# lgemc/WildlifeMapper

Measured on AMD Instinct MI355X. Metric: 1024x1024 tiles/sec (whole node), higher is better.
Workload: dtype fp16; 1 GPU; vit_h full path fft+encoder+decoder+PostProcess/NMS, fp16 MFMA, batch=16 tiles/GPU of 1024x1024x3 (BASELINE.json configs[2]); parallelism=dp1 tile shard, weights=seed 0 synthetic (random init), tolerance=logits within 1e-3 relative of the fp32 CPU forward, identical NMS index lists

## Files before the change

### include/wm_hip.h

```cpp
#ifndef WM_HIP_H
#define WM_HIP_H

#include <stdint.h>

#ifdef __cplusplus
extern "C" {
#endif

#define WM_ABI_VERSION 13

#define WM_PREC_BF16 0
#define WM_PREC_FP16 1
#define WM_PREC_FP8 2

#define WM_MAX_GLOBAL 8
#define WM_NUM_QUERIES 51
#define WM_NUM_LOGITS 8

typedef struct wm_config {
    int32_t embed_dim;
    int32_t depth;
    int32_t num_heads;
    int32_t num_global;
    int32_t global_attn_indexes[WM_MAX_GLOBAL];
// ... 236 lines not shown
                        float eps, void* out_16_dev, int M, int N, int K, int act, int precision, void* stream);
int wm_op_gemm16_stats(const void* a_dev, const void* w_dev, const float* bias_dev, const float* residual_dev, float* out_f32_dev,
                       void* x16_dev, float* stats_dev, int M, int N, int K, int layout, int precision, void* stream);
int wm_op_pack16(const void* in_dev, void* out_dev, int64_t rows, int K, void* stream);
int wm_op_unpack16(const void* in_dev, void* out_dev, int64_t rows, int K, void* stream);

int wm_op_ln_stats16_split(const float* x_dev, float* stats_dev, void* hi_dev, void* lo_dev, float* x_rw_dev, int64_t rows, int C,
                           int precision, void* stream);
int wm_op_gemm16_split(const void* a_dev, const void* w_dev, const float* bias_dev, void* hi_dev, void* lo_dev, float* stats_dev,
                       int M, int N, int K, int layout, int precision, void* stream);
int wm_op_stream_merge(const void* hi_dev, const void* lo_dev, float* out_dev, int64_t rows, int C, int precision, void* stream);

int wm_op_gemm8(const void* a_dev, const void* w_dev, const float* wscale_dev, const float* bias_dev,
                const float* residual_dev, float* out_f32_dev, void* out_16_dev, void* out_8_dev,
                int M, int N, int K, int act, int precision, void* stream);
int wm_op_stream_rows(float* x_f32_dev, void* hi_dev, void* lo_dev, int64_t rows, int C, int precision, int merge, void* stream);
int wm_op_gemm8_planes(const void* a_dev, const void* w_dev, const float* wscale_dev, const float* bias_dev, void* hi_dev, void* lo_dev,
                       int M, int N, int K, int precision, void* stream);
int wm_op_layernorm_fp8_plane(const void* hi_dev, const float* gamma_dev, const float* beta_dev, float eps, void* out_8_dev, int64_t rows, int C,
                              int precision, void* stream);
int wm_op_cvt_f32_to_fp8(const float* in_dev, void* out_dev, int64_t n, void* stream);

int wm_op_conv3x3_16(const void* a_dev, const void* w_dev, float* out_dev, int batch, int c_out, int c_in,
                     int precision, void* stream);

int wm_op_patch_embed16(const void* img16_dev, const void* w_dev, const float* bias_dev, float* out_f32_dev, void* out_16_dev,
                        int batch, int n_out, int c_in, int precision, void* stream);

#define WM_GEMM32_SPLIT 0x100
#define WM_GEMM32_PRESPLIT 0x200
int wm_op_gemm32(const float* a_dev, const float* w_dev, const float* bias_dev,
                 const float* residual_dev, float* out_dev, int M, int N, int K, int act, void* stream);

int wm_op_layernorm(const float* x_dev, const float* gamma_dev, const float* beta_dev, float eps,
                    float* out_f32_dev, void* out_16_dev, int64_t rows, int C, int precision, void* stream);

int wm_op_encoder_attention(const void* qkv_dev, const float* qkv_bias_dev,
                            const float* rel_pos_h_dev, const float* rel_pos_w_dev, void* out_dev,
                            int batch, int heads, int head_dim, int window, int precision, void* stream);

int wm_op_encoder_attention_qkv(const void* q_dev, const void* k_dev, const void* v_dev, int token_stride,
                                const float* qkv_bias_dev, const float* rel_pos_h_dev, const float* rel_pos_w_dev,
                                void* out_dev, int batch, int heads, int head_dim, int window, int precision, void* stream);

int wm_op_mha16(const void* q_dev, int q_stride, const void* k_dev, int k_stride,
                const void* v_dev, int v_stride, void* out_dev, int out_stride,
                int batch, int heads, int head_dim, int nq, int nk, int precision, void* stream);

int wm_op_mha32(const float* q_dev, const float* k_dev, const float* v_dev, float* out_dev,
                int batch, int heads, int head_dim, int nq, int nk, void* stream);

#ifdef __cplusplus
}
#endif
#endif
```

### wildlifemapper_amd/_native.py

```python
from __future__ import annotations

import ctypes as C
import os
from typing import Optional

import torch

_HERE = os.path.dirname(os.path.abspath(__file__))
LIB_PATH = os.environ.get("WM_HIP_LIB") or os.path.join(_HERE, "libwm_hip.so")

PREC_BF16, PREC_FP16, PREC_FP8 = 0, 1, 2
PREC_BY_NAME = {"bf16": PREC_BF16, "fp16": PREC_FP16, "f16": PREC_FP16, "fp8": PREC_FP8}
NUM_QUERIES, NUM_LOGITS = 51, 8
KCLASS_NAMES = ("gemm16", "attn_window", "attn_global", "layernorm", "other")
GEMM_VARIANTS = ("v1_128", "v2_160", "v2_128", "v3_lockstep", "v3_conv3x3", "v5_320", "v5_320_res", "v5_256", "v5_256_res",
                 "v5_320_lnf", "v5_256_lnf", "fp8_320", "fp8_256", "v5_320_foldp", "v5_256_foldp", "v5_320_split", "v5_256_split", "v3_patch_embed", "fp8_256_planes")
FLAG_CONF, FLAG_SCORE, FLAG_NMS, FLAG_MERGED = 1, 2, 4, 8
CRITERION_MAX_TARGETS, CRITERION_SUMS, CRITERION_NONFINITE, CRITERION_UNSOLVED = 2048, 8, 1, 2
CENSUS_MAX_DETS, CENSUS_SAME_CLASS, CENSUS_UNSOLVED = 262144, 1, 1
COVERAGE_MAX_SIDE, COVERAGE_MAX_CELLS, COVERAGE_MAX_FRAMES, COVERAGE_CLASSES, COVERAGE_STATS = 16384, 1 << 26, 65535, 7, 16
MOSAIC_NEAREST, MOSAIC_BILINEAR, MOSAIC_NORTH_UP = 0, 1, 1
MOSAIC_BAD_SLOT, MOSAIC_BAD_SIZE, MOSAIC_BAD_SOURCE = 1, 2, 4
REGISTER_MAX_SIDE, REGISTER_MAX_SEARCH, REGISTER_MAX_PAIRS = 512, 64, 65535
REGISTER_BAD_SLOT, REGISTER_BAD_SIZE, REGISTER_BAD_PAIR = 1, 2, 4
# ... 62 lines not shown
    "wm_criterion": (_I, [_P, _P, _P, _P, _P, C.POINTER(C.c_int32), _I, _F, _F, _F, _F, _P, _L, _P, _P, _P, _P, _P, _P, _P]),
    "wm_forward": (_I, [_P, _P, _P, _P, _P, _P, _I, _P]),
    "wm_set_tap": (_I, [_P, _I]),
    "wm_read_tap": (_I, [_P, _P, _I, _P]),
    "wm_profile_enable": (_I, [_P, _I]),
    "wm_profile_reset": (_I, [_P]),
    "wm_profile_read": (_I, [_P, C.POINTER(WmKclassStat)]),
    "wm_debug_gemm_variant_counts": (_I, [C.POINTER(_L), _I]),
    "wm_debug_reset_gemm_variant_counts": (_I, []),
    "wm_debug_saturation_enable": (_I, [_P, _I]),
    "wm_debug_saturation_read": (_I, [_P, C.POINTER(_L), _I, _I, _P]),
    "wm_op_cvt_f32_to_16": (_I, [_P, _P, _L, _I, _P]),
    "wm_op_cvt_16_to_f32": (_I, [_P, _P, _L, _I, _P]),
    "wm_op_gemm16": (_I, [_P, _P, _P, _P, _I, _P, _P, _I, _I, _I, _I, _I, _P]),
    "wm_op_gemm16_takes_packed": (_I, [_I, _I, _I]),
    "wm_op_pack16": (_I, [_P, _P, _L, _I, _P]),
    "wm_op_ln_stats16": (_I, [_P, _P, _P, _L, _I, _I, _P]),
    "wm_op_ln_stats16_split": (_I, [_P, _P, _P, _P, _P, _L, _I, _I, _P]),
    "wm_op_gemm16_split": (_I, [_P, _P, _P, _P, _P, _P, _I, _I, _I, _I, _I, _P]),
    "wm_op_stream_merge": (_I, [_P, _P, _P, _L, _I, _I, _P]),
    "wm_op_unpack16": (_I, [_P, _P, _L, _I, _P]),
    "wm_stream_overflow": (_I, [_P, _I]),
    "wm_op_fold_weight16": (_I, [_P, _P, _P, _P, _P, _P, _P, _I, _I, _I, _P]),
    "wm_op_gemm16_folded": (_I, [_P, _P, _P, _P, _P, _F, _P, _I, _I, _I, _I, _I, _P]),
    "wm_op_gemm16_stats": (_I, [_P, _P, _P, _P, _P, _P, _P, _I, _I, _I, _I, _I, _P]),
    "wm_op_gemm8": (_I, [_P, _P, _P, _P, _P, _P, _P, _P, _I, _I, _I, _I, _I, _P]),
    "wm_op_stream_rows": (_I, [_P, _P, _P, _L, _I, _I, _I, _P]),
    "wm_op_gemm8_planes": (_I, [_P, _P, _P, _P, _P, _P, _I, _I, _I, _I, _P]),
    "wm_op_layernorm_fp8_plane": (_I, [_P, _P, _P, _F, _P, _L, _I, _I, _P]),
    "wm_op_cvt_f32_to_fp8": (_I, [_P, _P, _L, _P]),
    "wm_op_conv3x3_16": (_I, [_P, _P, _P, _I, _I, _I, _I, _P]),
    "wm_op_patch_embed16": (_I, [_P, _P, _P, _P, _P, _I, _I, _I, _I, _P]),
    "wm_op_gemm32": (_I, [_P, _P, _P, _P, _P, _I, _I, _I, _I, _P]),
    "wm_op_layernorm": (_I, [_P, _P, _P, _F, _P, _P, _L, _I, _I, _P]),
    "wm_op_encoder_attention": (_I, [_P, _P, _P, _P, _P, _I, _I, _I, _I, _I, _P]),
    "wm_op_encoder_attention_qkv": (_I, [_P, _P, _P, _I, _P, _P, _P, _P, _I, _I, _I, _I, _I, _P]),
    "wm_op_mha16": (_I, [_P, _I, _P, _I, _P, _I, _P, _I, _I, _I, _I, _I, _I, _I, _P]),
    "wm_op_mha32": (_I, [_P, _P, _P, _P, _I, _I, _I, _I, _I, _P]),
}

_lib: Optional[C.CDLL] = None


def lib() -> C.CDLL:
    global _lib
    if _lib is None:
        if not os.path.exists(LIB_PATH):
            raise RuntimeError(
                f"{LIB_PATH} not found: build it with `python -c 'import __graft_entry__ as g; g.build()'` "
                "(hipcc --offload-arch=gfx950).  There is no CPU fallback.")
        l = C.CDLL(LIB_PATH)
        for name, (res, args) in SYMBOLS.items():
            fn = getattr(l, name)
            fn.restype = res
            fn.argtypes = args
        got = l.wm_abi_version()
        if got != ABI_VERSION:
            raise RuntimeError(f"{LIB_PATH} reports ABI version {got}, this binding was written for {ABI_VERSION}: "
                               "rebuild it (python -c 'import __graft_entry__ as g; g.build()')")
        _lib = l
    return _lib


def gemm_variant_counts(reset: bool = False) -> dict:
    arr = (C.c_int64 * len(GEMM_VARIANTS))()
    check(lib().wm_debug_gemm_variant_counts(arr, len(GEMM_VARIANTS)))
# ... 26 lines not shown
```

### wildlifemapper_amd/csrc/gemm32.h

```cpp
#pragma once
#include "wm_common.h"
#include "gemm_common.h"

namespace wm {

struct Gemm32Args {
    const float* A; const float* W; const float* bias; const float* residual; float* out;
    int M, N, K, act;
    int lda;
};

__global__ __launch_bounds__(256) void gemm32_kernel(Gemm32Args p) {
    constexpr int BM = 64, BN = 64, BK = 32, LD = BK + 1;
    __shared__ float sA[BM * LD];
    __shared__ float sW[BN * LD];
    const int tid = threadIdx.x, lane = tid & 63, wave = tid >> 6;
    const int wr = wave >> 1, wc = wave & 1;
    const int ntn = (p.N + BN - 1) / BN;
    const int lid = xcd_remap(blockIdx.x, gridDim.x);
    const int m0 = (lid / ntn) * BM, n0 = (lid % ntn) * BN;
    const int lrow = tid >> 2, lcol = (tid & 3) * 8;

    f32x16 acc;
#pragma unroll
// ... 126 lines not shown
        if (kt + 2 < nk) fetch(s, (kt + 2) * BK);
#pragma unroll
        for (int ks = 0; ks < 2; ++ks) {
            const typename FP16::vec8 a_hi = *(const typename FP16::vec8*)(sAh + fa + 16 * ks), a_lo = *(const typename FP16::vec8*)(sAl + fa + 16 * ks);
            const typename FP16::vec8 w_hi = *(const typename FP16::vec8*)(sWh + fw + 16 * ks), w_lo = *(const typename FP16::vec8*)(sWl + fw + 16 * ks);
            accx = FP16::mfma32(a_lo, w_hi, accx);
            accx = FP16::mfma32(a_hi, w_lo, accx);
            acc = FP16::mfma32(a_hi, w_hi, acc);
        }
    };
    for (int kt = 0; kt < nk; kt += 2) {
        step(st[0], kt);
        if (kt + 1 < nk) step(st[1], kt + 1);
    }
    if (amax >= 65504.f && p.overflow) *(volatile int*)p.overflow = 1;

    const int n = n0 + wc * 32 + (lane & 31);
    if (n >= p.N) return;
    const float bv = p.bias ? p.bias[n] : 0.f;
#pragma unroll
    for (int r = 0; r < 16; ++r) {
        const int m = m0 + wr * 32 + (r & 3) + 8 * (r >> 2) + 4 * (lane >> 5);
        if (m < p.M) {
            float v = (acc[r] + accx[r] * (1.0f / G32X3_LOSCALE)) * (1.0f / G32X3_WSCALE) + bv;
            if (p.act == ACT_RELU) v = fmaxf(v, 0.f);
            else if (p.act == ACT_GELU) v = gelu_erf(v);
            else if (p.act == ACT_SIGMOID) v = 1.0f / (1.0f + expf(-v));
            if (p.residual) v += p.residual[(size_t)m * p.N + n];
            p.out[(size_t)m * p.N + n] = v;
        }
    }
}

}
```

### wildlifemapper_amd/csrc/host_decoder.h

```cpp
#pragma once
#include "dec_kernels.h"
#include "host_encoder.h"

namespace {

struct DecAttnW { const float *wq, *bq, *wk, *bk, *wv, *bv, *wo, *bo; int internal; };

DecAttnW dec_w(wm_handle* h, const std::string& p, int internal) {
    return DecAttnW{W32(h, p + "q_proj.weight"), W32(h, p + "q_proj.bias"), W32(h, p + "k_proj.weight"), W32(h, p + "k_proj.bias"),
                    W32(h, p + "v_proj.weight"), W32(h, p + "v_proj.bias"), W32(h, p + "out_proj.weight"), W32(h, p + "out_proj.bias"), internal};
}

int decoder_impl(wm_handle* h, const float* keys_nhwc, float* logits, float* boxes, int B, hipStream_t s) {
    const std::string t = "mask_decoder.transformer.";
    const int E = OUTC, Mk = B * T, Mq = B * NQ;
    const float* tok = W32(h, "mask_decoder.mask_tokens.weight");
    float* keys = h->dkeys;
    HIP_TRY(hipMemcpyAsync(keys, keys_nhwc, (size_t)Mk * E * 4, hipMemcpyDeviceToDevice, s));
    float* queries = h->dq;
    WM_TRY(launch_simple(h, s, 0.0, add_bcast_kernel, dim3(grid_for((int64_t)Mq * E / 4)), dim3(256), (const float*)nullptr, tok, queries, (int64_t)Mq, E, NQ));

    auto add_q = [&](float* out) {
        return launch_simple(h, s, 0.0, add_bcast_kernel, dim3(grid_for((int64_t)Mq * E / 4)), dim3(256), (const float*)queries, tok, out, (int64_t)Mq, E, NQ);
    };
    auto add_k = [&](float* out) {
        return launch_simple(h, s, 0.0, add_bcast_kernel, dim3(grid_for((int64_t)Mk * E / 4)), dim3(256), (const float*)keys, (const float*)h->kpe, out, (int64_t)Mk, E, T);
    };
    auto ln = [&](float* x, const std::string& n, int rows) {
        return launch_layernorm(h, s, WM_PREC_FP16, x, W32(h, n + ".weight"), W32(h, n + ".bias"), 1e-5f, x, nullptr, rows, E);
    };
    auto token_to_image = [&](const DecAttnW& w, const float* kin) -> int {
        WM_TRY(add_q(h->dt_h1));
        WM_TRY(launch_gemm32(h, s, h->dt_h1, w.wq, w.bq, nullptr, h->dt_q, Mq, w.internal, E, ACT_NONE));
        WM_TRY(launch_gemm32(h, s, kin, w.wk, w.bk, nullptr, h->dk_a, Mk, w.internal, E, ACT_NONE));
        WM_TRY(launch_gemm32(h, s, keys, w.wv, w.bv, nullptr, h->dk_b, Mk, w.internal, E, ACT_NONE));
        WM_TRY(launch_mha32(h, s, h->dt_q, h->dk_a, h->dk_b, h->dt_att, B, 8, w.internal / 8, NQ, T));
        WM_TRY(launch_gemm32(h, s, h->dt_att, w.wo, w.bo, queries, queries, Mq, E, w.internal, ACT_NONE));
        return 0;
    };
    float* kpe_sum = h->n1;

    for (int i = 0; i < 2; ++i) {
        const std::string L = t + "layers." + std::to_string(i) + ".";
        {
            const DecAttnW w = dec_w(h, L + "self_attn.", E);
            const float* qin = queries;
            if (i != 0) { WM_TRY(add_q(h->dt_h1)); qin = h->dt_h1; }
            WM_TRY(launch_gemm32(h, s, qin, w.wq, w.bq, nullptr, h->dt_q, Mq, E, E, ACT_NONE));
            WM_TRY(launch_gemm32(h, s, qin, w.wk, w.bk, nullptr, h->dt_k, Mq, E, E, ACT_NONE));
            WM_TRY(launch_gemm32(h, s, queries, w.wv, w.bv, nullptr, h->dt_v, Mq, E, E, ACT_NONE));
            WM_TRY(launch_mha32(h, s, h->dt_q, h->dt_k, h->dt_v, h->dt_att, B, 8, E / 8, NQ, NQ));
            WM_TRY(launch_gemm32(h, s, h->dt_att, w.wo, w.bo, i == 0 ? nullptr : queries, queries, Mq, E, E, ACT_NONE));
            WM_TRY(ln(queries, L + "norm1", Mq));
        }
        WM_TRY(add_k(kpe_sum));
        WM_TRY(token_to_image(dec_w(h, L + "cross_attn_token_to_image.", E / 2), kpe_sum));
        WM_TRY(ln(queries, L + "norm2", Mq));
        WM_TRY(launch_gemm32(h, s, queries, W32(h, L + "mlp.lin1.weight"), W32(h, L + "mlp.lin1.bias"), nullptr, h->dt_hid, Mq, DEC_MLP, E, ACT_RELU));
        WM_TRY(launch_gemm32(h, s, h->dt_hid, W32(h, L + "mlp.lin2.weight"), W32(h, L + "mlp.lin2.bias"), queries, queries, Mq, E, DEC_MLP, ACT_NONE));
        WM_TRY(ln(queries, L + "norm3", Mq));
        {
            const DecAttnW w = dec_w(h, L + "cross_attn_image_to_token.", E / 2);
            WM_TRY(add_q(h->dt_h1));
            WM_TRY(launch_gemm32(h, s, kpe_sum, w.wq, w.bq, nullptr, h->dk_a, Mk, w.internal, E, ACT_NONE));
            WM_TRY(launch_gemm32(h, s, h->dt_h1, w.wk, w.bk, nullptr, h->dt_k, Mq, w.internal, E, ACT_NONE));
            WM_TRY(launch_gemm32(h, s, queries, w.wv, w.bv, nullptr, h->dt_v, Mq, w.internal, E, ACT_NONE));
            WM_TRY(launch_mha32(h, s, h->dk_a, h->dt_k, h->dt_v, h->dk_c, B, 8, w.internal / 8, T, NQ));
            WM_TRY(launch_gemm32(h, s, h->dk_c, w.wo, w.bo, keys, keys, Mk, E, w.internal, ACT_NONE));
            WM_TRY(ln(keys, L + "norm4", Mk));
        }
    }
    WM_TRY(add_k(kpe_sum));
    WM_TRY(token_to_image(dec_w(h, t + "final_attn_token_to_image.", E / 2), kpe_sum));
    WM_TRY(ln(queries, t + "norm_final_attn", Mq));

    const std::string c = "mask_decoder.class_embed.layers.", bb = "mask_decoder.bbox_embed.layers.";
    WM_TRY(launch_gemm32(h, s, queries, W32(h, c + "0.weight"), W32(h, c + "0.bias"), nullptr, h->dt_h1, Mq, E, E, ACT_RELU));
    WM_TRY(launch_gemm32(h, s, h->dt_h1, W32(h, c + "1.weight"), W32(h, c + "1.bias"), nullptr, h->dt_h2, Mq, E, E, ACT_RELU));
    WM_TRY(launch_gemm32(h, s, h->dt_h2, W32(h, c + "2.weight"), W32(h, c + "2.bias"), nullptr, logits, Mq, WM_NUM_LOGITS, E, ACT_NONE));
    WM_TRY(launch_gemm32(h, s, queries, W32(h, bb + "0.weight"), W32(h, bb + "0.bias"), nullptr, h->dt_h1, Mq, E, E, ACT_RELU));
    WM_TRY(launch_gemm32(h, s, h->dt_h1, W32(h, bb + "1.weight"), W32(h, bb + "1.bias"), nullptr, h->dt_h2, Mq, E, E, ACT_RELU));
    WM_TRY(launch_gemm32(h, s, h->dt_h2, W32(h, bb + "2.weight"), W32(h, bb + "2.bias"), nullptr, boxes, Mq, 4, E, ACT_SIGMOID));
    return 0;
}

int forward_impl(wm_handle* h, const float* x_dev, const float* target_sizes_dev, float* logits_dev, float* boxes_dev,
                 wm_box_record* records_dev, int batch, hipStream_t s) {
    WM_TRY(fft_impl(h, x_dev, h->hfc, batch, s, true));
    WM_TRY(encoder_impl(h, x_dev, h->hfc, nullptr, batch, s, true));
    WM_TRY(decoder_impl(h, h->emb_nhwc, h->logits, h->boxes, batch, s));
    const float* ts = target_sizes_dev ? target_sizes_dev : h->tsz_default;
    WM_TRY(launch_simple(h, s, 0.0, postprocess_nms_kernel, dim3(batch), dim3(64), (const float*)h->logits, (const float*)h->boxes, ts,
                         0.05f, 0.5f, 0.4f, h->records));
    if (logits_dev) HIP_TRY(hipMemcpyAsync(logits_dev, h->logits, (size_t)batch * NQ * WM_NUM_LOGITS * 4, hipMemcpyDeviceToDevice, s));
    if (boxes_dev) HIP_TRY(hipMemcpyAsync(boxes_dev, h->boxes, (size_t)batch * NQ * 16, hipMemcpyDeviceToDevice, s));
    if (records_dev) HIP_TRY(hipMemcpyAsync(records_dev, h->records, (size_t)batch * NQ * sizeof(wm_box_record), hipMemcpyDeviceToDevice, s));
    return 0;
}

}
```

### wildlifemapper_amd/csrc/host_gemm.h

```cpp
#pragma once
#include "gemm16.h"
#include "gemm16_v2.h"
#include "gemm16_v3.h"
#include "gemm16_v5.h"
#include "gemm32.h"
#include "gemm8.h"
#include "misc_kernels.h"
#include "host_core.h"

namespace {

double gemm16_flops(const Gemm16Args& a) { return 2.0 * a.M * (double)a.N * a.K; }
double gemm16_bytes(const Gemm16Args& a) {
    return 2.0 * ((double)a.M * a.K + (double)a.N * a.K) + (a.out32 ? 4.0 : 0.0) * a.M * a.N + (a.out16 ? 2.0 : 0.0) * a.M * a.N +
           (a.residual ? 4.0 * (double)(a.res_mod > 0 ? a.res_mod : a.M) * a.N : 0.0);
}

template <class Kern, class Args>
int launch_gemm_kernel(wm_handle* h, hipStream_t s, Kern kern, int grid, int threads, int lds, const Args& a, int variant, double flops, double bytes) {
    WM_TRY(set_max_lds((const void*)kern, lds));
    if (variant >= 0) count_variant(variant);
    Bracket br(h, s, WM_KCLASS_GEMM16, flops, bytes);
    hipLaunchKernelGGL(kern, dim3(grid), dim3(threads), lds, s, a);
    HIP_TRY(hipGetLastError());
    return 0;
}

template <class T16>
int launch_gemm16_t(wm_handle* h, hipStream_t s, const Gemm16Args& a) {
    return launch_gemm_kernel(h, s, gemm16_kernel<T16>, (a.M / G16_BM) * (a.N / G16_BN), 256, G16_LDS_BYTES, a, WM_GEMM_V1_128, gemm16_flops(a), gemm16_bytes(a));
}

template <class T16, int BN>
int launch_gemm16v2_t(wm_handle* h, hipStream_t s, const Gemm16Args& a) {
    return launch_gemm_kernel(h, s, gemm16v2_kernel<T16, BN>, (a.M / 256) * (a.N / BN), 512, G2<BN>::LDS, a, BN == 160 ? WM_GEMM_V2_160 : WM_GEMM_V2_128,
                              gemm16_flops(a), gemm16_bytes(a));
}

template <class T16, int BN, bool FOLDP, bool FOLDC, bool SPLIT, int NSLOT = 3>
int launch_gemm16v5_t(wm_handle* h, hipStream_t s, const Gemm16Args& a_in) {
    using G = G3<BN>;
// ... 133 lines not shown
    if (M % 4096 || N % 256 || Cin % 32) return fail("conv3x3: M=%d N=%d C=%d unsupported (M %% 4096, N %% 256, C %% 32)", M, N, Cin);
    const uint16_t* zero_page = nullptr;
    WM_TRY(zero_page_for_device(&zero_page));
    Gemm16Args a{};
    a.A = (const u16*)A; a.W = (const u16*)W; a.out32 = out32; a.M = M; a.N = N; a.K = 9 * Cin; a.act = ACT_NONE; a.conv_c = Cin; a.zero_page = (const u16*)zero_page;
    using G = G3<256>;
    count_variant(WM_GEMM_V3_CONV3X3);
    return by_type16(prec, [&](auto t) {
        return launch_gemm_kernel(h, s, gemm16v3_kernel<decltype(t), 256, ALoad::Conv3x3>, (M / 256) * (N / 256), G::THREADS, G::LDS, a, -1,
                                  2.0 * M * (double)N * 9 * Cin, 2.0 * ((double)M * Cin + 9.0 * N * Cin) + 4.0 * M * N);
    });
}

int launch_patch_embed16(wm_handle* h, hipStream_t s, int prec, const void* img16, const void* W, const float* bias, const float* res, int res_mod,
                         float* out32, void* out16, int B, int N, int Cin) {
    const int M = B * 4096, K = Cin * 256;
    if (B <= 0 || (N % 320 && N % 256) || Cin <= 0) return fail("patch_embed: B=%d N=%d Cin=%d unsupported (N %% 320 or N %% 256)", B, N, Cin);
    if (!out32 && !out16) return fail("patch_embed: no output");
    Gemm16Args a{};
    a.A = (const u16*)img16; a.W = (const u16*)W; a.bias = bias; a.residual = res; a.out32 = out32; a.out16 = (u16*)out16;
    a.M = M; a.N = N; a.K = K; a.res_mod = res_mod; a.act = ACT_NONE; a.conv_c = Cin;
    count_variant(WM_GEMM_V3_PATCH);
    const double bytes = 2.0 * ((double)M * K + (double)N * K) + (out32 ? 4.0 : 0.0) * M * N + (out16 ? 2.0 : 0.0) * M * N;
    return by_type16(prec, [&](auto t) {
        return by_tile_width(N, [&](auto bn) {
            constexpr int BN = decltype(bn)::value;
            using G = G3<BN>;
            return launch_gemm_kernel(h, s, gemm16v3_kernel<decltype(t), BN, ALoad::PatchEmbed>, (M / 256) * (N / BN), G::THREADS, G::LDS, a, -1,
                                      2.0 * M * (double)N * K, bytes);
        });
    });
}

int launch_gemm32(wm_handle* h, hipStream_t s, const float* A, const float* W, const float* bias, const float* res,
                  float* out, int M, int N, int K, int act, int lda = 0, int mode = 0) {
    if (K % 16) return fail("gemm32: K=%d must be a multiple of 16", K);
    static const bool f32_only = getenv("WM_GEMM32_F32") && atoi(getenv("WM_GEMM32_F32")) != 0;
    if ((mode == 2 || mode == 3) && K % 32) return fail("gemm32 (split form): K=%d must be a multiple of 32", K);
    if (mode == 2 || mode == 3 || (mode == 0 && h && !f32_only && K % 32 == 0)) {
        Gemm32x3Args a{A, W, nullptr, nullptr, bias, res, out, M, N, K, act, lda > 0 ? lda : K, h ? h->overflow + 1 : nullptr};
        if (mode == 3) {
            const size_t n = (size_t)N * K;
            void* pb = nullptr;
            WM_TRY(op_scratch(s, 3, n * 4, &pb));
            u16* hi = (u16*)pb;
            hipLaunchKernelGGL(split_w32_kernel, dim3(grid_for((int64_t)n / 4)), dim3(256), 0, s, W, hi, hi + n, (int64_t)n / 4, (int*)nullptr);
            HIP_TRY(hipGetLastError());
            a.Whi = hi; a.Wlo = hi + n;
        }
        if (mode == 0) {
            auto it = h->w32x3.find(W);
            if (it == h->w32x3.end()) {
                uint16_t *hi = nullptr, *lo = nullptr;
                const size_t n = (size_t)N * K;
                if (n % 4) return fail("gemm32: weight of %zu elements", n);
                WM_TRY(dalloc(h, &hi, n * 2)); WM_TRY(dalloc(h, &lo, n * 2));
                hipLaunchKernelGGL(split_w32_kernel, dim3(grid_for((int64_t)n / 4)), dim3(256), 0, s, W, (u16*)hi, (u16*)lo, (int64_t)n / 4, h->overflow + 1);
                HIP_TRY(hipGetLastError());
                it = h->w32x3.emplace(W, std::make_pair(hi, lo)).first;
            }
            a.Whi = (const u16*)it->second.first; a.Wlo = (const u16*)it->second.second;
        }
        Bracket br(h, s, WM_KCLASS_OTHER, 2.0 * M * (double)N * K, 4.0 * ((double)M * K + (double)M * N) + 4.0 * (double)N * K);
        const dim3 grid(((N + 63) / 64) * ((M + 63) / 64));
        if (mode == 0 || mode == 3) hipLaunchKernelGGL(gemm32x3_kernel<true>, grid, dim3(256), 0, s, a);
        else hipLaunchKernelGGL(gemm32x3_kernel<false>, grid, dim3(256), 0, s, a);
        HIP_TRY(hipGetLastError());
        return 0;
    }
    Gemm32Args a{A, W, bias, res, out, M, N, K, act, lda > 0 ? lda : K};
    Bracket br(h, s, WM_KCLASS_OTHER, 2.0 * M * (double)N * K, 4.0 * ((double)M * K + (double)N * K + (double)M * N));
    hipLaunchKernelGGL(gemm32_kernel, dim3(((N + 63) / 64) * ((M + 63) / 64)), dim3(256), 0, s, a);
    HIP_TRY(hipGetLastError());
    return 0;
}

}
```

### wildlifemapper_amd/csrc/wm_api.hip

```cpp
#include "host_core.h"
#if WM_DEV_TIMELINE
#include "host_dev_timeline.h"
#endif
#include "host_gemm.h"
#include "host_norm.h"
#include "host_attn.h"
#include "host_weights.h"
#include "host_encoder.h"
#include "host_decoder.h"
#include "host_frontend.h"
#include "host_criterion.h"

extern "C" const char* wm_last_error(void) { return g_err; }
extern "C" int wm_abi_version(void) { return WM_ABI_VERSION; }

extern "C" int wm_create(const wm_config* cfg, int device, wm_handle** out) {
    if (!cfg || !out) return fail("wm_create: null argument");
    if (cfg->embed_dim <= 0 || cfg->num_heads <= 0 || cfg->embed_dim % cfg->num_heads) return fail("wm_create: bad dims");
    if (cfg->depth <= 0 || cfg->depth > 64) return fail("wm_create: depth %d out of range", cfg->depth);
    if (cfg->max_batch <= 0) return fail("wm_create: max_batch must be positive");
    if (cfg->embed_dim % 256 || cfg->embed_dim > 1280) return fail("wm_create: embed_dim %d unsupported (multiple of 256, <= 1280)", cfg->embed_dim);
    const int hd = cfg->embed_dim / cfg->num_heads;
    if (hd != 64 && hd != 80) return fail("wm_create: head_dim %d unsupported (64 or 80)", hd);
    if (cfg->precision != WM_PREC_BF16 && cfg->precision != WM_PREC_FP16 && cfg->precision != WM_PREC_FP8) return fail("wm_create: bad precision");
// ... 430 lines not shown
                        hi_dev, lo_dev);
}

extern "C" int wm_op_layernorm_fp8_plane(const void* hi_dev, const float* gamma_dev, const float* beta_dev, float eps, void* out_8_dev, int64_t rows, int C,
                                        int precision, void* stream) {
    if (!hi_dev || !out_8_dev || !gamma_dev || !beta_dev) return fail("wm_op_layernorm_fp8_plane: null buffer");
    return launch_layernorm_plane8(nullptr, (hipStream_t)stream, precision, hi_dev, gamma_dev, beta_dev, eps, out_8_dev, rows, C);
}

extern "C" int wm_op_cvt_f32_to_fp8(const float* in_dev, void* out_dev, int64_t n, void* stream) {
    if (n % 4) return fail("cvt fp8: n must be a multiple of 4");
    return launch_simple(nullptr, (hipStream_t)stream, 0.0, cvt_f32_to_fp8_kernel, dim3(grid_for(n / 4)), dim3(256), in_dev, (unsigned char*)out_dev, n / 4);
}

extern "C" int wm_op_conv3x3_16(const void* a_dev, const void* w_dev, float* out_dev, int batch, int c_out, int c_in, int precision,
                               void* stream) {
    return launch_conv3x3_16(nullptr, (hipStream_t)stream, precision, a_dev, w_dev, out_dev, batch * 4096, c_out, c_in);
}

extern "C" int wm_op_patch_embed16(const void* img16_dev, const void* w_dev, const float* bias_dev, float* out_f32_dev, void* out_16_dev,
                                  int batch, int n_out, int c_in, int precision, void* stream) {
    if (!img16_dev || !w_dev) return fail("wm_op_patch_embed16: null buffer");
    return launch_patch_embed16(nullptr, (hipStream_t)stream, precision, img16_dev, w_dev, bias_dev, nullptr, 0, out_f32_dev, out_16_dev, batch, n_out, c_in);
}

extern "C" int wm_op_gemm32(const float* a_dev, const float* w_dev, const float* bias_dev, const float* residual_dev, float* out_dev,
                            int M, int N, int K, int act, void* stream) {
    const int split = (act & WM_GEMM32_SPLIT) != 0, presplit = (act & WM_GEMM32_PRESPLIT) != 0;
    if (split && presplit) return fail("wm_op_gemm32: WM_GEMM32_SPLIT and WM_GEMM32_PRESPLIT are exclusive");
    return launch_gemm32(nullptr, (hipStream_t)stream, a_dev, w_dev, bias_dev, residual_dev, out_dev, M, N, K, act & 0xff, 0,
                         presplit ? 3 : split ? 2 : 1);
}

extern "C" int wm_op_layernorm(const float* x_dev, const float* gamma_dev, const float* beta_dev, float eps, float* out_f32_dev,
                               void* out_16_dev, int64_t rows, int C, int precision, void* stream) {
    const int packed = (precision & WM_LAYOUT_PACKED) != 0;
    precision &= ~WM_LAYOUT_PACKED;
    if (!out_f32_dev && out_16_dev)
        return launch_layernorm_block(nullptr, (hipStream_t)stream, precision, x_dev, gamma_dev, beta_dev, eps, out_16_dev, rows, C, packed);
    if (packed) return fail("wm_op_layernorm: the LDS-image-order output exists for the 16-bit-only form");
    return launch_layernorm(nullptr, (hipStream_t)stream, precision, x_dev, gamma_dev, beta_dev, eps, out_f32_dev, out_16_dev, rows, C);
}

extern "C" int wm_op_encoder_attention(const void* qkv_dev, const float* qkv_bias_dev, const float* rel_pos_h_dev,
                                       const float* rel_pos_w_dev, void* out_dev, int batch, int heads, int head_dim, int window,
                                       int precision, void* stream) {
    return launch_encoder_attention(nullptr, (hipStream_t)stream, precision, qkv_dev, qkv_bias_dev, rel_pos_h_dev, rel_pos_w_dev, out_dev,
                                    batch, heads, head_dim, window);
}

extern "C" int wm_op_encoder_attention_qkv(const void* q_dev, const void* k_dev, const void* v_dev, int token_stride, const float* qkv_bias_dev,
                                           const float* rel_pos_h_dev, const float* rel_pos_w_dev, void* out_dev, int batch, int heads,
                                           int head_dim, int window, int precision, void* stream) {
    AttnExtra x;
    x.k_sep = k_dev; x.v_sep = v_dev; x.tok_stride = token_stride;
    return launch_encoder_attention(nullptr, (hipStream_t)stream, precision, q_dev, qkv_bias_dev, rel_pos_h_dev, rel_pos_w_dev, out_dev,
                                    batch, heads, head_dim, window, x);
}

extern "C" int wm_op_mha16(const void* q_dev, int q_stride, const void* k_dev, int k_stride, const void* v_dev, int v_stride,
                           void* out_dev, int out_stride, int batch, int heads, int head_dim, int nq, int nk, int precision, void* stream) {
    return launch_mha16(nullptr, (hipStream_t)stream, precision, q_dev, q_stride, k_dev, k_stride, v_dev, v_stride, out_dev, out_stride,
                        batch, heads, head_dim, nq, nk);
}

extern "C" int wm_op_mha32(const float* q_dev, const float* k_dev, const float* v_dev, float* out_dev, int batch, int heads,
// ... 4 lines not shown
```

Before: 173.2 tiles/s.

## Fuse positional-embedding add and norm4 LayerNorm into row-block fp32x3 decoder GEMMs

Adds a row-blocked split-fp16 GEMM kernel that covers the full N (128 or 256) per block. It can add a broadcast positional embedding to A while loading, and can apply LayerNorm to the output rows in the epilogue. The decoder now uses it for key projections, which drops the separate add_k kernels and the kpe_sum buffer. It also folds the norm4 LayerNorm into the output projection and removes the initial device-to-device copy of the keys. The decoder is a small part of the vit_h pipeline, so the gain is likely small, and the fused epilogue may change rounding slightly.

```diff
diff --git a/include/wm_hip.h b/include/wm_hip.h
--- a/include/wm_hip.h
+++ b/include/wm_hip.h
@@ -292,6 +292,11 @@
 int wm_op_gemm32(const float* a_dev, const float* w_dev, const float* bias_dev,
                  const float* residual_dev, float* out_dev, int M, int N, int K, int act, void* stream);
 
+int wm_op_gemm32_rows(const float* a_dev, const float* pos_dev, int pos_rows, const float* w_dev, const float* bias_dev,
+                      const float* residual_dev, float* out_dev, const float* ln_gamma_dev, const float* ln_beta_dev, float ln_eps,
+                      int M, int N, int K, int act, void* stream);
+int wm_op_gemm32_takes_rows(int M, int N, int K);
+
 int wm_op_layernorm(const float* x_dev, const float* gamma_dev, const float* beta_dev, float eps,
                     float* out_f32_dev, void* out_16_dev, int64_t rows, int C, int precision, void* stream);
 
diff --git a/wildlifemapper_amd/_native.py b/wildlifemapper_amd/_native.py
--- a/wildlifemapper_amd/_native.py
+++ b/wildlifemapper_amd/_native.py
@@ -118,6 +118,8 @@
     "wm_op_conv3x3_16": (_I, [_P, _P, _P, _I, _I, _I, _I, _P]),
     "wm_op_patch_embed16": (_I, [_P, _P, _P, _P, _P, _I, _I, _I, _I, _P]),
     "wm_op_gemm32": (_I, [_P, _P, _P, _P, _P, _I, _I, _I, _I, _P]),
+    "wm_op_gemm32_rows": (_I, [_P, _P, _I, _P, _P, _P, _P, _P, _P, _F, _I, _I, _I, _I, _P]),
+    "wm_op_gemm32_takes_rows": (_I, [_I, _I, _I]),
     "wm_op_layernorm": (_I, [_P, _P, _P, _F, _P, _P, _L, _I, _I, _P]),
     "wm_op_encoder_attention": (_I, [_P, _P, _P, _P, _P, _I, _I, _I, _I, _I, _P]),
     "wm_op_encoder_attention_qkv": (_I, [_P, _P, _P, _I, _P, _P, _P, _P, _I, _I, _I, _I, _I, _P]),
diff --git a/wildlifemapper_amd/csrc/gemm32.h b/wildlifemapper_amd/csrc/gemm32.h
--- a/wildlifemapper_amd/csrc/gemm32.h
+++ b/wildlifemapper_amd/csrc/gemm32.h
@@ -182,4 +182,170 @@
     }
 }
 
-}
+struct Gemm32RowsArgs {
+    const float* A; const float* pos; const u16* Whi; const u16* Wlo;
+    const float* bias; const float* residual; float* out;
+    const float* ln_g; const float* ln_b; float ln_eps;
+    int M, N, K, act, lda, pos_rows;
+    int* overflow;
+};
+
+template <int I, int N, class F>
+__device__ __forceinline__ void g32_static_for(F&& f) {
+    if constexpr (I < N) {
+        f(std::integral_constant<int, I>{});
+        g32_static_for<I + 1, N>(f);
+    }
+}
+
+template <int NJ>
+struct G32Rows {
+    static constexpr int BM = 64, BK = 32, LDH = BK + 8, N = 64 * NJ;
+    static constexpr int LDO = N + 4;
+    static constexpr int LOOP_BYTES = (2 * BM + 2 * N) * LDH * 2, EPI_BYTES = BM * LDO * 4;
+    static constexpr int LDS = LOOP_BYTES > EPI_BYTES ? LOOP_BYTES : EPI_BYTES;
+};
+
+template <int NJ, bool LN>
+__global__ __launch_bounds__(256, NJ == 2 ? 3 : 2) void gemm32x3_rows_kernel(Gemm32RowsArgs p) {
+    using G = G32Rows<NJ>;
+    constexpr int BM = G::BM, BK = G::BK, LDH = G::LDH, N = G::N, LDO = G::LDO;
+    static_assert(!LN || NJ == 4, "the fused LayerNorm is the 256-column form: one wave per row");
+    extern __shared__ __attribute__((aligned(16))) unsigned char g32r_lds[];
+    u16* const sAh = (u16*)g32r_lds;
+    u16* const sAl = sAh + BM * LDH;
+    u16* const sWh = sAl + BM * LDH;
+    u16* const sWl = sWh + N * LDH;
+    float* const sO = (float*)g32r_lds;
+    const int tid = threadIdx.x, lane = tid & 63, wave = tid >> 6;
+    const int wr = wave >> 1, wc = wave & 1;
+    const int m0 = blockIdx.x * BM;
+    const int lrow = tid >> 2, lcol = (tid & 3) * 8;
+
+    f32x16 acc[NJ], accx[NJ];
+#pragma unroll
+    for (int j = 0; j < NJ; ++j)
+#pragma unroll
+        for (int r = 0; r < 16; ++r) acc[j][r] = accx[j][r] = 0.f;
+    const float* ap = p.A + (size_t)(m0 + lrow) * p.lda + lcol;
+    const float* pp = p.pos ? p.pos + (size_t)((m0 + lrow) % p.pos_rows) * p.K + lcol : nullptr;
+    const size_t woff = (size_t)lrow * p.K + lcol;
+    struct AStage { f32x4 a0, a1, p0, p1; };
+    AStage st[2];
+    f16x8 wh[NJ], wl[NJ];
+    float amax = 0.f;
+    auto fetch_a = [&](AStage& s, int k0) {
+        s.a0 = *(const f32x4*)(ap + k0); s.a1 = *(const f32x4*)(ap + k0 + 4);
+        if (pp) { s.p0 = *(const f32x4*)(pp + k0); s.p1 = *(const f32x4*)(pp + k0 + 4); }
+    };
+    auto fetch_w = [&](int k0) {
+        g32_static_for<0, NJ>([&](auto ic) {
+            constexpr int i = decltype(ic)::value;
+            wh[i] = *(const f16x8*)(p.Whi + woff + (size_t)i * 64 * p.K + k0);
+            wl[i] = *(const f16x8*)(p.Wlo + woff + (size_t)i * 64 * p.K + k0);
+        });
+    };
+    auto split8 = [&](const f32x4& x0, const f32x4& x1, uint4& hi, uint4& lo) {
+        union { uint4 raw; typename FP16::vec4 h[2]; } uh, ul;
+#pragma unroll
+        for (int j = 0; j < 8; ++j) {
+            const float x = j < 4 ? x0[j] : x1[j - 4];
+            amax = fmaxf(amax, fabsf(x));
+            uh.h[j >> 2][j & 3] = FP16::from_f32_bounded(x);
+            ul.h[j >> 2][j & 3] = FP16::from_f32_bounded((x - FP16::to_f32(uh.h[j >> 2][j & 3])) * G32X3_LOSCALE);
+        }
+        hi = uh.raw; lo = ul.raw;
+    };
+    const int nk = p.K / BK;
+    fetch_a(st[0], 0);
+    fetch_w(0);
+    if (nk > 1) fetch_a(st[1], BK);
+    const int fa = (wr * 32 + (lane & 31)) * LDH + 8 * (lane >> 5), fw = (wc * NJ * 32 + (lane & 31)) * LDH + 8 * (lane >> 5);
+    auto step = [&](AStage& s, int kt) {
+        uint4 ah, al;
+        if (pp) split8(s.a0 + s.p0, s.a1 + s.p1, ah, al);
+        else split8(s.a0, s.a1, ah, al);
+        __syncthreads();
+        *(uint4*)(sAh + lrow * LDH + lcol) = ah; *(uint4*)(sAl + lrow * LDH + lcol) = al;
+        g32_static_for<0, NJ>([&](auto ic) {
+            constexpr int i = decltype(ic)::value;
+            *(f16x8*)(sWh + (i * 64 + lrow) * LDH + lcol) = wh[i];
+            *(f16x8*)(sWl + (i * 64 + lrow) * LDH + lcol) = wl[i];
+        });
+        __syncthreads();
+        if (kt + 1 < nk) fetch_w((kt + 1) * BK);
+        if (kt + 2 < nk) fetch_a(s, (kt + 2) * BK);
+#pragma unroll
+        for (int ks = 0; ks < 2; ++ks) {
+            const typename FP16::vec8 a_hi = *(const typename FP16::vec8*)(sAh + fa + 16 * ks), a_lo = *(const typename FP16::vec8*)(sAl + fa + 16 * ks);
+#pragma unroll
+            for (int j = 0; j < NJ; ++j) {
+                const typename FP16::vec8 w_hi = *(const typename FP16::vec8*)(sWh + fw + j * 32 * LDH + 16 * ks);
+                const typename FP16::vec8 w_lo = *(const typename FP16::vec8*)(sWl + fw + j * 32 * LDH + 16 * ks);
+                accx[j] = FP16::mfma32(a_lo, w_hi, accx[j]);
+                accx[j] = FP16::mfma32(a_hi, w_lo, accx[j]);
+                acc[j] = FP16::mfma32(a_hi, w_hi, acc[j]);
+            }
+        }
+    };
+    for (int kt = 0; kt < nk; kt += 2) {
+        step(st[0], kt);
+        if (kt + 1 < nk) step(st[1], kt + 1);
+    }
+    if (amax >= 65504.f && p.overflow) *(volatile int*)p.overflow = 1;
+
+    __syncthreads();
+#pragma unroll
+    for (int j = 0; j < NJ; ++j) {
+        const int n = (wc * NJ + j) * 32 + (lane & 31);
+        const float bv = p.bias ? p.bias[n] : 0.f;
+#pragma unroll
+        for (int r = 0; r < 16; ++r) {
+            const int row = wr * 32 + (r & 3) + 8 * (r >> 2) + 4 * (lane >> 5);
+            float v = (acc[j][r] + accx[j][r] * (1.0f / G32X3_LOSCALE)) * (1.0f / G32X3_WSCALE) + bv;
+            if (p.act == ACT_RELU) v = fmaxf(v, 0.f);
+            else if (p.act == ACT_GELU) v = gelu_erf(v);
+            else if (p.act == ACT_SIGMOID) v = 1.0f / (1.0f + expf(-v));
+            sO[row * LDO + n] = v;
+        }
+    }
+    constexpr int LPR = N / 4, RPI = 64 / LPR, NIT = 16 / RPI;
+    const int c0 = (lane % LPR) * 4, row0 = wave * 16 + lane / LPR;
+    f32x4 rv[NIT], g, b;
+    if (p.residual) {
+#pragma unroll
+        for (int it = 0; it < NIT; ++it) rv[it] = *(const f32x4*)(p.residual + (size_t)(m0 + row0 + it * RPI) * N + c0);
+    }
+    if constexpr (LN) {
+        g = *(const f32x4*)(p.ln_g + c0);
+        b = *(const f32x4*)(p.ln_b + c0);
+    }
+    __syncthreads();
+#pragma unroll
+    for (int it = 0; it < NIT; ++it) {
+        const int row = row0 + it * RPI;
+        const size_t o = (size_t)(m0 + row) * N + c0;
+        f32x4 v = *(const f32x4*)(sO + row * LDO + c0);
+        if (p.residual) v += rv[it];
+        if constexpr (LN) {
+            float sum = 0.f;
+            sum += (v[0] + v[1]) + (v[2] + v[3]);
+            const float mean = wave_sum(sum) * (1.0f / N);
+            float sq = 0.f;
+#pragma unroll
+            for (int j = 0; j < 4; ++j) {
+                const float d = v[j] - mean;
+                sq += d * d;
+            }
+            const float var = wave_sum(sq) * (1.0f / N);
+            const float rstd = 1.0f / sqrtf(var + p.ln_eps);
+            f32x4 y;
+#pragma unroll
+            for (int j = 0; j < 4; ++j) y[j] = (v[j] - mean) * rstd * g[j] + b[j];
+            v = y;
+        }
+        *(f32x4*)(p.out + o) = v;
+    }
+}
+
+}
diff --git a/wildlifemapper_amd/csrc/host_decoder.h b/wildlifemapper_amd/csrc/host_decoder.h
--- a/wildlifemapper_amd/csrc/host_decoder.h
+++ b/wildlifemapper_amd/csrc/host_decoder.h
@@ -15,31 +15,27 @@
     const std::string t = "mask_decoder.transformer.";
     const int E = OUTC, Mk = B * T, Mq = B * NQ;
     const float* tok = W32(h, "mask_decoder.mask_tokens.weight");
-    float* keys = h->dkeys;
-    HIP_TRY(hipMemcpyAsync(keys, keys_nhwc, (size_t)Mk * E * 4, hipMemcpyDeviceToDevice, s));
+    const float* keys = keys_nhwc;
     float* queries = h->dq;
     WM_TRY(launch_simple(h, s, 0.0, add_bcast_kernel, dim3(grid_for((int64_t)Mq * E / 4)), dim3(256), (const float*)nullptr, tok, queries, (int64_t)Mq, E, NQ));
 
     auto add_q = [&](float* out) {
         return launch_simple(h, s, 0.0, add_bcast_kernel, dim3(grid_for((int64_t)Mq * E / 4)), dim3(256), (const float*)queries, tok, out, (int64_t)Mq, E, NQ);
     };
-    auto add_k = [&](float* out) {
-        return launch_simple(h, s, 0.0, add_bcast_kernel, dim3(grid_for((int64_t)Mk * E / 4)), dim3(256), (const float*)keys, (const float*)h->kpe, out, (int64_t)Mk, E, T);
-    };
+    Gemm32RowsExtra with_pe;
+    with_pe.pos = h->kpe; with_pe.pos_rows = T; with_pe.pos_scratch = h->n1;
     auto ln = [&](float* x, const std::string& n, int rows) {
         return launch_layernorm(h, s, WM_PREC_FP16, x, W32(h, n + ".weight"), W32(h, n + ".bias"), 1e-5f, x, nullptr, rows, E);
     };
-    auto token_to_image = [&](const DecAttnW& w, const float* kin) -> int {
+    auto token_to_image = [&](const DecAttnW& w) -> int {
         WM_TRY(add_q(h->dt_h1));
         WM_TRY(launch_gemm32(h, s, h->dt_h1, w.wq, w.bq, nullptr, h->dt_q, Mq, w.internal, E, ACT_NONE));
-        WM_TRY(launch_gemm32(h, s, kin, w.wk, w.bk, nullptr, h->dk_a, Mk, w.internal, E, ACT_NONE));
-        WM_TRY(launch_gemm32(h, s, keys, w.wv, w.bv, nullptr, h->dk_b, Mk, w.internal, E, ACT_NONE));
+        WM_TRY(launch_gemm32_rows(h, s, keys, w.wk, w.bk, nullptr, h->dk_a, Mk, w.internal, E, ACT_NONE, with_pe));
+        WM_TRY(launch_gemm32_rows(h, s, keys, w.wv, w.bv, nullptr, h->dk_b, Mk, w.internal, E, ACT_NONE, Gemm32RowsExtra{}));
         WM_TRY(launch_mha32(h, s, h->dt_q, h->dk_a, h->dk_b, h->dt_att, B, 8, w.internal / 8, NQ, T));
         WM_TRY(launch_gemm32(h, s, h->dt_att, w.wo, w.bo, queries, queries, Mq, E, w.internal, ACT_NONE));
         return 0;
     };
-    float* kpe_sum = h->n1;
-
     for (int i = 0; i < 2; ++i) {
         const std::string L = t + "layers." + std::to_string(i) + ".";
         {
@@ -53,8 +49,7 @@
             WM_TRY(launch_gemm32(h, s, h->dt_att, w.wo, w.bo, i == 0 ? nullptr : queries, queries, Mq, E, E, ACT_NONE));
             WM_TRY(ln(queries, L + "norm1", Mq));
         }
-        WM_TRY(add_k(kpe_sum));
-        WM_TRY(token_to_image(dec_w(h, L + "cross_attn_token_to_image.", E / 2), kpe_sum));
+        WM_TRY(token_to_image(dec_w(h, L + "cross_attn_token_to_image.", E / 2)));
         WM_TRY(ln(queries, L + "norm2", Mq));
         WM_TRY(launch_gemm32(h, s, queries, W32(h, L + "mlp.lin1.weight"), W32(h, L + "mlp.lin1.bias"), nullptr, h->dt_hid, Mq, DEC_MLP, E, ACT_RELU));
         WM_TRY(launch_gemm32(h, s, h->dt_hid, W32(h, L + "mlp.lin2.weight"), W32(h, L + "mlp.lin2.bias"), queries, queries, Mq, E, DEC_MLP, ACT_NONE));
@@ -62,16 +57,17 @@
         {
             const DecAttnW w = dec_w(h, L + "cross_attn_image_to_token.", E / 2);
             WM_TRY(add_q(h->dt_h1));
-            WM_TRY(launch_gemm32(h, s, kpe_sum, w.wq, w.bq, nullptr, h->dk_a, Mk, w.internal, E, ACT_NONE));
+            WM_TRY(launch_gemm32_rows(h, s, keys, w.wq, w.bq, nullptr, h->dk_a, Mk, w.internal, E, ACT_NONE, with_pe));
             WM_TRY(launch_gemm32(h, s, h->dt_h1, w.wk, w.bk, nullptr, h->dt_k, Mq, w.internal, E, ACT_NONE));
             WM_TRY(launch_gemm32(h, s, queries, w.wv, w.bv, nullptr, h->dt_v, Mq, w.internal, E, ACT_NONE));
             WM_TRY(launch_mha32(h, s, h->dk_a, h->dt_k, h->dt_v, h->dk_c, B, 8, w.internal / 8, T, NQ));
-            WM_TRY(launch_gemm32(h, s, h->dk_c, w.wo, w.bo, keys, keys, Mk, E, w.internal, ACT_NONE));
-            WM_TRY(ln(keys, L + "norm4", Mk));
+            Gemm32RowsExtra norm4;
+            norm4.ln_g = W32(h, L + "norm4.weight"); norm4.ln_b = W32(h, L + "norm4.bias"); norm4.ln_eps = 1e-5f;
+            WM_TRY(launch_gemm32_rows(h, s, h->dk_c, w.wo, w.bo, keys, h->dkeys, Mk, E, w.internal, ACT_NONE, norm4));
+            keys = h->dkeys;
         }
     }
-    WM_TRY(add_k(kpe_sum));
-    WM_TRY(token_to_image(dec_w(h, t + "final_attn_token_to_image.", E / 2), kpe_sum));
+    WM_TRY(token_to_image(dec_w(h, t + "final_attn_token_to_image.", E / 2)));
     WM_TRY(ln(queries, t + "norm_final_attn", Mq));
 
     const std::string c = "mask_decoder.class_embed.layers.", bb = "mask_decoder.bbox_embed.layers.";
diff --git a/wildlifemapper_amd/csrc/host_gemm.h b/wildlifemapper_amd/csrc/host_gemm.h
--- a/wildlifemapper_amd/csrc/host_gemm.h
+++ b/wildlifemapper_amd/csrc/host_gemm.h
@@ -6,7 +6,9 @@
 #include "gemm32.h"
 #include "gemm8.h"
 #include "misc_kernels.h"
+#include "dec_kernels.h"
 #include "host_core.h"
+#include "host_norm.h"
 
 namespace {
 
@@ -206,6 +208,30 @@
     });
 }
 
+static int gemm32_w_planes(wm_handle* h, hipStream_t s, const float* W, int N, int K, const u16** whi, const u16** wlo) {
+    const size_t n = (size_t)N * K;
+    if (n % 4) return fail("gemm32: weight of %zu elements", n);
+    if (!h) {
+        void* pb = nullptr;
+        WM_TRY(op_scratch(s, 3, n * 4, &pb));
+        u16* hi = (u16*)pb;
+        hipLaunchKernelGGL(split_w32_kernel, dim3(grid_for((int64_t)n / 4)), dim3(256), 0, s, W, hi, hi + n, (int64_t)n / 4, (int*)nullptr);
+        HIP_TRY(hipGetLastError());
+        *whi = hi; *wlo = hi + n;
+        return 0;
+    }
+    auto it = h->w32x3.find(W);
+    if (it == h->w32x3.end()) {
+        uint16_t *hi = nullptr, *lo = nullptr;
+        WM_TRY(dalloc(h, &hi, n * 2)); WM_TRY(dalloc(h, &lo, n * 2));
+        hipLaunchKernelGGL(split_w32_kernel, dim3(grid_for((int64_t)n / 4)), dim3(256), 0, s, W, (u16*)hi, (u16*)lo, (int64_t)n / 4, h->overflow + 1);
+        HIP_TRY(hipGetLastError());
+        it = h->w32x3.emplace(W, std::make_pair(hi, lo)).first;
+    }
+    *whi = (const u16*)it->second.first; *wlo = (const u16*)it->second.second;
+    return 0;
+}
+
 int launch_gemm32(wm_handle* h, hipStream_t s, const float* A, const float* W, const float* bias, const float* res,
                   float* out, int M, int N, int K, int act, int lda = 0, int mode = 0) {
     if (K % 16) return fail("gemm32: K=%d must be a multiple of 16", K);
@@ -213,28 +239,7 @@
     if ((mode == 2 || mode == 3) && K % 32) return fail("gemm32 (split form): K=%d must be a multiple of 32", K);
     if (mode == 2 || mode == 3 || (mode == 0 && h && !f32_only && K % 32 == 0)) {
         Gemm32x3Args a{A, W, nullptr, nullptr, bias, res, out, M, N, K, act, lda > 0 ? lda : K, h ? h->overflow + 1 : nullptr};
-        if (mode == 3) {
-            const size_t n = (size_t)N * K;
-            void* pb = nullptr;
-            WM_TRY(op_scratch(s, 3, n * 4, &pb));
-            u16* hi = (u16*)pb;
-            hipLaunchKernelGGL(split_w32_kernel, dim3(grid_for((int64_t)n / 4)), dim3(256), 0, s, W, hi, hi + n, (int64_t)n / 4, (int*)nullptr);
-            HIP_TRY(hipGetLastError());
-            a.Whi = hi; a.Wlo = hi + n;
-        }
-        if (mode == 0) {
-            auto it = h->w32x3.find(W);
-            if (it == h->w32x3.end()) {
-                uint16_t *hi = nullptr, *lo = nullptr;
-                const size_t n = (size_t)N * K;
-                if (n % 4) return fail("gemm32: weight of %zu elements", n);
-                WM_TRY(dalloc(h, &hi, n * 2)); WM_TRY(dalloc(h, &lo, n * 2));
-                hipLaunchKernelGGL(split_w32_kernel, dim3(grid_for((int64_t)n / 4)), dim3(256), 0, s, W, (u16*)hi, (u16*)lo, (int64_t)n / 4, h->overflow + 1);
-                HIP_TRY(hipGetLastError());
-                it = h->w32x3.emplace(W, std::make_pair(hi, lo)).first;
-            }
-            a.Whi = (const u16*)it->second.first; a.Wlo = (const u16*)it->second.second;
-        }
+        if (mode == 0 || mode == 3) WM_TRY(gemm32_w_planes(mode == 0 ? h : nullptr, s, W, N, K, &a.Whi, &a.Wlo));
         Bracket br(h, s, WM_KCLASS_OTHER, 2.0 * M * (double)N * K, 4.0 * ((double)M * K + (double)M * N) + 4.0 * (double)N * K);
         const dim3 grid(((N + 63) / 64) * ((M + 63) / 64));
         if (mode == 0 || mode == 3) hipLaunchKernelGGL(gemm32x3_kernel<true>, grid, dim3(256), 0, s, a);
@@ -249,4 +254,53 @@
     return 0;
 }
 
-}
+struct Gemm32RowsExtra {
+    const float* pos = nullptr;
+    int pos_rows = 0;
+    float* pos_scratch = nullptr;
+    const float* ln_g = nullptr;
+    const float* ln_b = nullptr;
+    float ln_eps = 0.f;
+};
+static bool gemm32_takes_rows(int M, int N, int K) { return M >= 4096 && M % 128 == 0 && (N == 128 || N == 256) && K > 0 && K % 32 == 0; }
+static bool aligned16(const void* p) { return ((uintptr_t)p & 15) == 0; }
+
+int launch_gemm32_rows(wm_handle* h, hipStream_t s, const float* A, const float* W, const float* bias, const float* res, float* out,
+                       int M, int N, int K, int act, const Gemm32RowsExtra& x) {
+    if (x.pos && x.pos_rows <= 0) return fail("gemm32 (rows): pos_rows=%d", x.pos_rows);
+    if ((x.ln_g != nullptr) != (x.ln_b != nullptr)) return fail("gemm32 (rows): LayerNorm takes both gamma and beta");
+    if (x.ln_g && N != 256) return fail("gemm32 (rows): the LayerNorm option is for N = 256, not %d", N);
+    static const bool f32_only = getenv("WM_GEMM32_F32") && atoi(getenv("WM_GEMM32_F32")) != 0;
+    const bool ptrs = aligned16(A) && aligned16(x.pos) && aligned16(res) && aligned16(out) && aligned16(x.ln_g) && aligned16(x.ln_b);
+    if (gemm32_takes_rows(M, N, K) && ptrs && !(h && f32_only)) {
+        Gemm32RowsArgs a{A, x.pos, nullptr, nullptr, bias, res, out, x.ln_g, x.ln_b, x.ln_eps, M, N, K, act, K, x.pos_rows, h ? h->overflow + 1 : nullptr};
+        WM_TRY(gemm32_w_planes(h, s, W, N, K, &a.Whi, &a.Wlo));
+        auto go = [&](auto kern, int lds) {
+            WM_TRY(set_max_lds((const void*)kern, lds));
+            Bracket br(h, s, WM_KCLASS_OTHER, 2.0 * M * (double)N * K,
+                       4.0 * ((double)M * K + (double)M * N * (res ? 2.0 : 1.0) + (double)N * K + (x.pos ? (double)x.pos_rows * K : 0.0)));
+            hipLaunchKernelGGL(kern, dim3(M / 64), dim3(256), lds, s, a);
+            HIP_TRY(hipGetLastError());
+            return 0;
+        };
+        if (N == 128) return go(gemm32x3_rows_kernel<2, false>, G32Rows<2>::LDS);
+        return x.ln_g ? go(gemm32x3_rows_kernel<4, true>, G32Rows<4>::LDS) : go(gemm32x3_rows_kernel<4, false>, G32Rows<4>::LDS);
+    }
+    const float* a_in = A;
+    if (x.pos) {
+        float* sum = x.pos_scratch;
+        if (!sum) {
+            void* pb = nullptr;
+            WM_TRY(op_scratch(s, 4, (size_t)M * K * 4, &pb));
+            sum = (float*)pb;
+        }
+        if (K % 4) return fail("gemm32 (rows): K=%d", K);
+        WM_TRY(launch_simple(h, s, 0.0, add_bcast_kernel, dim3(grid_for((int64_t)M * K / 4)), dim3(256), A, x.pos, sum, (int64_t)M, K, x.pos_rows));
+        a_in = sum;
+    }
+    WM_TRY(launch_gemm32(h, s, a_in, W, bias, res, out, M, N, K, act, 0, h ? 0 : 3));
+    if (x.ln_g) WM_TRY(launch_layernorm(h, s, WM_PREC_FP16, out, x.ln_g, x.ln_b, x.ln_eps, out, nullptr, M, N));
+    return 0;
+}
+
+}
diff --git a/wildlifemapper_amd/csrc/wm_api.hip b/wildlifemapper_amd/csrc/wm_api.hip
--- a/wildlifemapper_amd/csrc/wm_api.hip
+++ b/wildlifemapper_amd/csrc/wm_api.hip
@@ -486,6 +486,17 @@
                          presplit ? 3 : split ? 2 : 1);
 }
 
+extern "C" int wm_op_gemm32_rows(const float* a_dev, const float* pos_dev, int pos_rows, const float* w_dev, const float* bias_dev,
+                                 const float* residual_dev, float* out_dev, const float* ln_gamma_dev, const float* ln_beta_dev, float ln_eps,
+                                 int M, int N, int K, int act, void* stream) {
+    if (!a_dev || !w_dev || !out_dev || M <= 0 || N <= 0 || K <= 0) return fail("wm_op_gemm32_rows: null buffer or empty shape");
+    Gemm32RowsExtra x;
+    x.pos = pos_dev; x.pos_rows = pos_rows; x.ln_g = ln_gamma_dev; x.ln_b = ln_beta_dev; x.ln_eps = ln_eps;
+    return launch_gemm32_rows(nullptr, (hipStream_t)stream, a_dev, w_dev, bias_dev, residual_dev, out_dev, M, N, K, act, x);
+}
+
+extern "C" int wm_op_gemm32_takes_rows(int M, int N, int K) { return gemm32_takes_rows(M, N, K) ? 1 : 0; }
+
 extern "C" int wm_op_layernorm(const float* x_dev, const float* gamma_dev, const float* beta_dev, float eps, float* out_f32_dev,
                                void* out_16_dev, int64_t rows, int C, int precision, void* stream) {
     const int packed = (precision & WM_LAYOUT_PACKED) != 0;
```

Result: no change. 173.8 tiles/s (median of 6 runs) (+0.3%).
